# wangsibovictor/fora

Hardware: AMD Instinct MI355X
Metric: SSPPR queries/sec at eps=0.5 (higher is better)
Workload: dtype u64 fixed-point 2^-62 (f64 at the boundary)

## Files before the change

### fora_amd/csrc/fora_kernels.h

```cpp
#pragma once
#include <hip/hip_runtime.h>
#include <stdint.h>
#include <type_traits>
#include "fora_diag.h"

namespace fora {

constexpr int BLOCK = 256;
constexpr uint32_t PUSH_SEG = 256;
constexpr uint32_t WALK_SEG = 1024;
#ifndef FORA_TEST_PATHS
#define FORA_TEST_PATHS 0
#endif
constexpr bool TEST_PATHS = FORA_TEST_PATHS != 0;
constexpr uint64_t FIX_ONE = 1ull << 62;
constexpr uint32_t DEG_SAT = 0xFFFFFFu;
constexpr int MAX_LEVELS = 1 << 15;
#ifndef FORA_BIN_SHIFT
#define FORA_BIN_SHIFT 13
#endif
constexpr int BIN_SHIFT = FORA_BIN_SHIFT;
constexpr uint32_t BIN_SIZE = 1u << BIN_SHIFT;
#ifndef FORA_BIN_SHIFT_WIDE
#define FORA_BIN_SHIFT_WIDE 14
// ... 216 lines not shown
    if (r2 < 0) { q2--; r2 += b; }
    if (r2 >= (int64_t)b) { q2++; }
    return q1 + (uint64_t)q2;
}

__device__ __forceinline__ uint64_t node_thr(uint64_t t1, uint32_t deg) {
    if (deg == 0) return 1;
    uint64_t hi = __umul64hi(t1, (uint64_t)deg);
    return hi ? ~0ull : t1 * (uint64_t)deg;
}

__device__ __forceinline__ uint64_t pop_value(uint64_t afix, uint64_t r, uint32_t deg, uint64_t &res_add, uint64_t &dang) {
    const uint64_t keep = mulshift62(r, afix);
    const uint64_t push = r - keep;
    if (deg == 0) { res_add = keep; dang = push; return 0; }
    const uint64_t inc = div_u64_u32(push, deg);
    res_add = keep + (push - inc * deg);
    dang = 0;
    return inc;
}

__device__ __forceinline__ uint64_t thr_unit(uint64_t t1, uint32_t k) {
    return k == 0 ? t1 : ((t1 >> (63 - k)) ? (~0ull >> 1) : (t1 << k));
}

__device__ __forceinline__ void node_row(const Dev &d, uint32_t v, int64_t &beg, uint64_t &deg) {
    uint64_t ri = d.rowinfo[v];
    beg = (int64_t)(ri >> 24);
    deg = ri & DEG_SAT;
    if (deg == DEG_SAT) deg = (uint64_t)(d.row_ptr[v + 1] - beg);
}

__device__ __forceinline__ uint32_t ri_deg(const Dev &d, uint64_t ri, uint32_t v) {
    const uint32_t dg = (uint32_t)ri & DEG_SAT;
    return dg == DEG_SAT ? (uint32_t)(d.row_ptr[v + 1] - (int64_t)(ri >> 24)) : dg;
}

struct __attribute__((packed, aligned(4))) U32Pair { uint32_t a, b; };
__device__ __forceinline__ uint32_t colp_at(const Dev &d, uint64_t e) {
    uint32_t word, sh;
    if (d.colp32) {
        const uint32_t at = d.colbits * (uint32_t)e;
        word = at >> 5; sh = at & 31;
    } else {
        const uint64_t at = (uint64_t)d.colbits * e;
        word = (uint32_t)(at >> 5); sh = (uint32_t)at & 31;
    }
    const U32Pair cw = *(const U32Pair *)(d.colp + word);
    const uint64_t both = ((uint64_t)cw.b << 32) | cw.a;
    return (uint32_t)(both >> sh) & ((1u << d.colbits) - 1u);
}
__device__ __forceinline__ uint32_t walk_move(const Dev &d, uint32_t cur, uint32_t start, uint32_t wm) {
    if (d.rp32) {
        const U32Pair rp = *(const U32Pair *)(d.rp32 + cur);
        const uint32_t dg = rp.b - rp.a;
        if (!dg) return start;
        return colp_at(d, (uint64_t)rp.a + __umulhi(wm, dg));
    }
    int64_t beg; uint64_t deg;
    node_row(d, cur, beg, deg);
    if (!deg) return start;
    return (uint32_t)d.col[beg + (int64_t)(((uint64_t)wm * deg) >> 32)];
}

__device__ __forceinline__ uint64_t wave_sum(uint64_t v) {
#pragma unroll
    for (int o = 32; o; o >>= 1) v += __shfl_xor(v, o);
    return v;
}
template <int CTRL, int ROWS = 0xF>
__device__ __forceinline__ uint32_t dpp0(uint32_t x) { return (uint32_t)__builtin_amdgcn_update_dpp(0, (int)x, CTRL, ROWS, 0xF, false); }
__device__ __forceinline__ uint32_t wave_incl_scan_add(uint32_t x) {
    x += dpp0<0x111>(x); x += dpp0<0x112>(x); x += dpp0<0x114>(x); x += dpp0<0x118>(x);
    x += dpp0<0x142, 0xA>(x);
    x += dpp0<0x143, 0xC>(x);
    return x;
}
__device__ __forceinline__ uint32_t wave_incl_scan_max(uint32_t x) {
    x = max(x, dpp0<0x111>(x)); x = max(x, dpp0<0x112>(x)); x = max(x, dpp0<0x114>(x)); x = max(x, dpp0<0x118>(x));
    x = max(x, dpp0<0x142, 0xA>(x));
    x = max(x, dpp0<0x143, 0xC>(x));
    return x;
}
__device__ __forceinline__ uint32_t wave_excl_scan(uint32_t v, uint32_t &total) {
    const uint32_t x = wave_incl_scan_add(v);
    total = (uint32_t)__builtin_amdgcn_readlane((int)x, 63);
    return x - v;
}
template <int NT>
__device__ __forceinline__ uint32_t block_excl_scan_n(uint32_t v, uint32_t *s_w, uint32_t &total) {
    uint32_t wtot;
    uint32_t x = wave_excl_scan(v, wtot);
    const int w = threadIdx.x >> 6;
    __syncthreads();
    if ((threadIdx.x & 63) == 0) s_w[w] = wtot;
    __syncthreads();
    uint32_t before = 0, tot = 0;
#pragma unroll
    for (int i = 0; i < NT / 64; i++) { const uint32_t c = s_w[i]; if (i < w) before += c; tot += c; }
    total = tot;
    return x + before;
}
__device__ __forceinline__ uint32_t block_excl_scan(uint32_t v, uint32_t *s_w, uint32_t &total) {
    uint32_t wtot;
    uint32_t x = wave_excl_scan(v, wtot);
    const int w = threadIdx.x >> 6;
    __syncthreads();
    if ((threadIdx.x & 63) == 0) s_w[w] = wtot;
    __syncthreads();
    uint32_t a0 = s_w[0], a1 = s_w[1], a2 = s_w[2], a3 = s_w[3];
    total = a0 + a1 + a2 + a3;
    return x + (w > 0 ? a0 : 0) + (w > 1 ? a1 : 0) + (w > 2 ? a2 : 0);
}

constexpr int ilog2(int x) { return x <= 1 ? 0 : 1 + ilog2(x >> 1); }
template <int NT>
__device__ __forceinline__ uint32_t pref_find(const uint32_t *s_pref, uint32_t x) {
    static_assert((NT & (NT - 1)) == 0, "a power of two entries");
    uint32_t lo = 0, hi = NT;
#pragma unroll
    for (int it = 0; it < ilog2(NT); it++) {
        const uint32_t mid = (lo + hi) >> 1;
        if (s_pref[mid] <= x) lo = mid; else hi = mid;
    }
    return lo;
}
__device__ __forceinline__ uint32_t pref_step(const uint32_t *s_pref, uint32_t lo, uint32_t x) {
    while (s_pref[lo + 1] <= x) lo++;
    return lo;
}

template <typename T>
__device__ __forceinline__ void slab_load(uint64_t (&x)[SLAB_UNROLL], const uint64_t *p, T base, T v0, T step, T n) {
#pragma unroll
    for (int u = 0; u < SLAB_UNROLL; u++) x[u] = v0 + u * step < n ? p[base + v0 + u * step] : 0;
}

__device__ __forceinline__ void wave_append(bool flag, uint64_t item, uint64_t *list,
                                            unsigned long long *count, uint64_t cap, uint32_t *err,
                                            uint32_t errbit) {
    const unsigned long long mask = __ballot(flag);
    if (!mask) return;
    const int lane = threadIdx.x & 63;
    const int leader = __ffsll((long long)mask) - 1;
    unsigned long long base = 0;
    if (lane == leader) base = atomicAdd(count, (unsigned long long)__popcll(mask));
    base = __shfl(base, leader);
    if (flag) {
        uint64_t idx = base + __popcll(mask & ((1ull << lane) - 1));
        if (idx < cap) list[idx] = item;
        else atomicOr(err, errbit);
    }
}

__device__ __forceinline__ void wave_append32(bool flag, uint32_t item, uint32_t *list, uint32_t *count,
                                              uint32_t cap, uint32_t *err, uint32_t errbit) {
    const unsigned long long mask = __ballot(flag);
    if (!mask) return;
    const int lane = threadIdx.x & 63;
    const int leader = __ffsll((long long)mask) - 1;
    uint32_t base = 0;
    if (lane == leader) base = atomicAdd(count, (uint32_t)__popcll(mask));
    base = __shfl(base, leader);
    if (flag) {
        const uint32_t idx = base + __popcll(mask & ((1ull << lane) - 1));
        if (idx < cap) list[idx] = item;
// ... 1580 lines not shown
    }
    if (__ballot(bad) && (threadIdx.x & 63) == 0) atomicOr(&fail[q], 2u);
}
__global__ void __launch_bounds__(BLOCK) k_bounds_reset(int32_t n, double *upper, double *lower) {
    const uint64_t slab = (uint64_t)blockIdx.y * n;
    for (uint64_t v = (uint64_t)blockIdx.x * BLOCK + threadIdx.x; v < (uint64_t)n; v += (uint64_t)gridDim.x * BLOCK) {
        upper[slab + v] = 1.0;
        lower[slab + v] = 0.0;
    }
}

__global__ void __launch_bounds__(BLOCK) k_index_alloc(Dev d) {
    const int lane = threadIdx.x & 63;
    const int q = 0;
    const uint32_t nchunk = ((uint32_t)d.n + BLOCK - 1) / BLOCK;
    for (uint32_t c = blockIdx.x; c < nchunk; c += gridDim.x) {
        const uint32_t v = c * BLOCK + threadIdx.x;
        uint64_t num = 0, ioff = 0;
        if (v < (uint32_t)d.n) { num = d.idx_cnt[v]; ioff = d.idx_off[v]; }
        const uint32_t nseg = (uint32_t)((num + WALK_SEG - 1) / WALK_SEG);
        uint32_t tot;
        const uint32_t off = wave_excl_scan(nseg, tot);
        if (tot) {
            uint32_t sb = 0;
            if (lane == 0) sb = atomicAdd(&d.wit_count[q * CSTRIDE], tot);
            sb = __shfl(sb, 0);
            if ((uint64_t)sb + tot > d.wit_cap) {
                if (lane == 0) atomicOr(d.err, ERR_WIT_OVERFLOW);
            } else {
                for (uint32_t k = 0; k < nseg; k++) {
                    WalkItem w = {};
                    w.j0 = (uint64_t)k * WALK_SEG;
                    const uint64_t left = num - w.j0;
                    w.cnt = left < WALK_SEG ? (uint32_t)left : WALK_SEG;
                    w.idx_pos = ioff + w.j0;
                    w.v = v;
                    d.wit[sb + off + k] = wit_pack(w);
                }
            }
        }
    }
}

enum { WALK_TO_PPR = 0, WALK_TO_INDEX = 1 };

__device__ __forceinline__ int32_t walk_one(const Dev &d, uint32_t start, uint64_t j, uint32_t stream,
                                            uint32_t round, int nzh, uint32_t &steps) {
    int64_t beg; uint64_t deg;
    node_row(d, start, beg, deg);
    if (deg == 0) return (int32_t)start;
    uint32_t cur = start;
    uint32_t w[4];
    for (uint32_t t = 0;; t++) {
        if ((t & 1u) == 0)
            philox4x32_10(start, (uint32_t)j,
                          (uint32_t)((j >> 32) & 0xFFFFu) | ((round & 0xFFu) << 16) | (((t >> 1) & 0xFFu) << 24),
                          stream ^ ((t >> 9) * 0x9E3779B9u), d.seed_lo, d.seed_hi, w);
        const uint32_t ws = (t & 1u) ? w[2] : w[0], wm = (t & 1u) ? w[3] : w[1];
        if (!(nzh && t == 0) && ws < d.alpha32) return (int32_t)cur;
        if (t) node_row(d, cur, beg, deg);
        if (deg > 0)
            cur = (uint32_t)d.col[beg + (int64_t)(((uint64_t)wm * deg) >> 32)];
        else
            cur = start;
        steps++;
    }
}

#ifndef FORA_STAGE
#define FORA_STAGE 320
#endif
#ifndef FORA_WALK_WPE
#define FORA_WALK_WPE 6
#endif
constexpr int STAGE = FORA_STAGE;
struct WaveStage {
    uint64_t *pk;
    uint32_t *bcnt;
    uint32_t *bbase;
    uint32_t *fill;
    uint32_t count;
    const uint32_t *xl;
};
template <int ST>
__device__ __forceinline__ void stage_flush(const Dev &d, int q, WaveStage &st) {
    const int lane = threadIdx.x & 63;
    const uint64_t slab = (uint64_t)q * d.n;
    const uint64_t bk0 = SubBuckets::first_of(d.pbins, d.sub, d.bk_cap, q, blockIdx.x), bstride = SubBuckets::stride_of(d.sub, d.bk_cap);
    st.bcnt[lane] = 0;
    st.bcnt[lane + 64] = 0;
    __builtin_amdgcn_wave_barrier();
    constexpr uint64_t NONE = ~0ull;
    uint32_t rk[ST / 64];
    uint64_t wv[ST / 64];
#pragma unroll
    for (int k = 0; k < ST / 64; k++) {
        const uint32_t m = k * 64 + lane;
        wv[k] = NONE;
        if (m < st.count) {
            wv[k] = st.pk[m];
            rk[k] = atomicAdd(&st.bcnt[((uint32_t)wv[k] & ((1u << WPACK_SHIFT) - 1)) >> BIN_SHIFT], 1u);
        }
    }
    __builtin_amdgcn_wave_barrier();
    {
        const uint32_t c0 = lane < d.nbins ? st.bcnt[lane] : 0, c1 = lane + 64 < d.nbins ? st.bcnt[lane + 64] : 0;
        uint32_t t0, t1;
        const uint32_t o0 = wave_excl_scan(c0, t0), o1 = wave_excl_scan(c1, t1);
        if (c0) st.bbase[lane] = atomicAdd(&st.fill[lane], c0);
        if (c1) st.bbase[lane + 64] = atomicAdd(&st.fill[lane + 64], c1);
        st.bcnt[lane] = o0;
        st.bcnt[lane + 64] = t0 + o1;
    }
    __builtin_amdgcn_wave_barrier();
#pragma unroll
    for (int k = 0; k < ST / 64; k++)
        if (wv[k] != NONE) st.pk[st.bcnt[((uint32_t)wv[k] & ((1u << WPACK_SHIFT) - 1)) >> BIN_SHIFT] + rk[k]] = wv[k];
    __builtin_amdgcn_wave_barrier();
#pragma unroll
    for (int k = 0; k < ST / 64; k++) {
        const uint32_t m = k * 64 + lane;
        if (m < st.count) {
            const uint64_t pk = st.pk[m];
            const uint32_t dd = (uint32_t)pk & ((1u << WPACK_SHIFT) - 1);
            const uint32_t b = dd >> BIN_SHIFT;
            const uint32_t pos = st.bbase[b] + (m - st.bcnt[b]);
            if (pos < d.bk_cap) __builtin_nontemporal_store(pk, &d.bk_inc[bk0 + (uint64_t)b * bstride + pos]);
            else atomicAdd((unsigned long long *)&d.ppr[slab + (st.xl ? st.xl[dd] : dd)], (unsigned long long)(pk >> WPACK_SHIFT));
        }
    }
    __builtin_amdgcn_wave_barrier();
    st.count = 0;
}
template <int ST>
__device__ __forceinline__ void stage_emit(const Dev &d, int q, WaveStage &st, bool has, uint32_t dest, uint64_t w) {
    if (has && w >= WPACK_MAXW) {
        atomicAdd((unsigned long long *)&d.ppr[(uint64_t)q * d.n + (st.xl ? st.xl[dest] : dest)], (unsigned long long)w);
        has = false;
    }
    const unsigned long long mask = __ballot(has);
    if (!mask) return;
    if (has) {
        const uint32_t pos = st.count + __popcll(mask & ((1ull << (threadIdx.x & 63)) - 1));
        st.pk[pos] = (uint64_t)dest | (w << WPACK_SHIFT);
    }
    st.count += (uint32_t)__popcll(mask);
    if (st.count > ST - 64) stage_flush<ST>(d, q, st);
}
#define WAVE_STAGE_DECL_N(st, NWAVES, ST)                                                           \
    __shared__ uint64_t st##_pk[NWAVES][ST];                                                        \
    __shared__ uint32_t st##_bcnt[NWAVES][MAX_BINS], st##_bbase[NWAVES][MAX_BINS];                 \
    __shared__ uint32_t st##_fill[MAX_BINS];                                                        \
    WaveStage st;                                                                                   \
    st.pk = st##_pk[threadIdx.x >> 6];                                                              \
    st.bcnt = st##_bcnt[threadIdx.x >> 6]; st.bbase = st##_bbase[threadIdx.x >> 6];                 \
    st.fill = st##_fill; st.count = 0; st.xl = nullptr;
#define WAVE_STAGE_DECL(st) WAVE_STAGE_DECL_N(st, BLOCK / 64, STAGE)

template <int NB>
__global__ void __launch_bounds__(BinThreads<NB>::value) k_walk_idx(Dev d) {
    constexpr int NT = BinThreads<NB>::value;
    constexpr int EPT = NB > MAX_BINS ? FORA_IDX_EPT_WIDE : BIN_EPT;
    constexpr uint32_t CHUNK = NT * EPT;
    constexpr uint32_t PAD = NB > MAX_BINS ? FORA_RUN_PAD_WIDE : 1;
    constexpr bool BINNED = NB > 1;
    constexpr bool WIDE = NB > MAX_BINS;
    constexpr int BS = WIDE ? BIN_SHIFT_WIDE : BIN_SHIFT;
    constexpr uint32_t BSZ = 1u << BS;
    constexpr int IB = NT == 256 ? 8 : NT == 512 ? 9 : 10;
    constexpr int DB = WIDE ? BS : WPACK_SHIFT;
    static_assert(DB + IB + 1 <= 32, "stage word: destination | item | carries-one-more-unit");
    __shared__ uint64_t s_j0[NT], s_pos[NT], s_incr[NT], s_rem[NT];
    __shared__ uint32_t s_pref[NT + 1], s_w[NT / 64];
    __shared__ uint32_t s_cnt[NB], s_lofs[NB + 1], s_fill[NB];
    __shared__ uint32_t s_msg[BINNED ? CHUNK : 1];
    __shared__ uint16_t s_bin[BINNED ? CHUNK : 1];
    const bool slot_major = NB > MAX_BINS && (d.slot_major & 4u);
    const int q = slot_major ? blockIdx.x : blockIdx.y;
    const uint32_t bx = slot_major ? blockIdx.y : blockIdx.x, gx = slot_major ? gridDim.y : gridDim.x;
    const uint32_t nitems = (uint32_t)min((uint64_t)d.wit_count[q * CSTRIDE], d.wit_cap);
    if (!nitems || *d.err) return;
    const WalkItemP *items = d.wit + (uint64_t)q * d.wit_cap;
    const uint64_t slab = (uint64_t)q * d.n;
    const uint32_t bin_lo = (uint32_t)d.bin_lo;
    const BinExchange<NB, NT, PAD> ex{s_cnt, s_lofs, s_fill, s_w, SubBuckets(d.bk_count, d.pbins, d.sub, d.bk_cap, q, bx), (uint32_t)d.bin_cnt};
    if (BINNED) ex.load_fills();
    constexpr uint32_t GRAN = FORA_TILE_GRAN_WALK;
    const uint32_t ntiles = (nitems + NT - 1) / NT;
    const uint32_t seg_len = ntiles * GRAN;
    for (uint32_t tile = bx; tile < ntiles; tile += gx) {
        const uint32_t i = tile_pos<GRAN>(threadIdx.x, tile, seg_len);
        uint32_t cnt = 0;
        if (i < nitems) {
            const WalkItem w = wit_load(&items[i]);
            s_j0[threadIdx.x] = w.j0; s_pos[threadIdx.x] = w.idx_pos;
            s_incr[threadIdx.x] = w.incr; s_rem[threadIdx.x] = w.rem;
            cnt = w.idx_n;
        }
        uint32_t total;
        const uint32_t pre = block_excl_scan_n<NT>(cnt, s_w, total);
        s_pref[threadIdx.x] = pre;
        if (threadIdx.x == 0) s_pref[NT] = total;
        __syncthreads();
        for (uint32_t cb = 0; cb < total; cb += CHUNK) {
            uint32_t dest[EPT], rank[EPT], li[EPT];
            const uint32_t e0 = cb + threadIdx.x * EPT;
            uint32_t lo = e0 < total ? pref_find<NT>(s_pref, e0) : 0;
#pragma unroll
            for (int k = 0; k < EPT; k++) {
                const uint32_t e = e0 + k;
                if (e < total) lo = pref_step(s_pref, lo, e);
                li[k] = lo;
            }
#pragma unroll
            for (int k = 0; k < EPT; k++) {
                const uint32_t e = e0 + k;
                dest[k] = 0xFFFFFFFFu;
                if (e < total) {
                    const uint32_t jj = e - s_pref[li[k]];
                    dest[k] = (uint32_t)d.rw_idx[s_pos[li[k]] + jj];
                    li[k] |= (s_j0[li[k]] + jj < s_rem[li[k]] ? 1u : 0u) << IB;
                }
            }
            if (!BINNED) {
#pragma unroll
                for (int k = 0; k < EPT; k++)
                    if (dest[k] != 0xFFFFFFFFu)
                        atomicAdd((unsigned long long *)&d.ppr[slab + dest[k]],
                                  (unsigned long long)(s_incr[li[k] & (NT - 1)] + (li[k] >> IB)));
                continue;
// ... 114 lines not shown
                    }
                    const uint32_t want = (uint32_t)__popcll(idle);
                    wptr += want < avail ? want : avail;
                    while (wptr < wend && s_pref[cur_item + 1] <= wptr) cur_item++;
                }
                if (active)
                    philox4x32_10(start, (uint32_t)wj,
                                  (uint32_t)((wj >> 32) & 0xFFFFu) | ((round & 0xFFu) << 16) | (((t >> 1) & 0xFFu) << 24),
                                  stream ^ ((t >> 9) * 0x9E3779B9u), d.seed_lo, d.seed_hi, rw);
            }
            if (active) {
                const uint32_t ws = (it & 1u) ? rw[2] : rw[0], wm = (it & 1u) ? rw[3] : rw[1];
                if (!(nzh && t == 0) && ws < d.alpha32) {
                    done = (int32_t)cur;
                    active = false;
                } else {
                    if (t) cur = walk_move(d, cur, start, wm);
                    else if (d.rp32) cur = colp_at(d, (uint64_t)beg0 + (((uint64_t)wm * deg0) >> 32));
                    else cur = (uint32_t)d.col[beg0 + (int64_t)(((uint64_t)wm * deg0) >> 32)];
                    t++;
                    steps++;
                }
            }
            if (staged) {
                stage_emit<STAGE>(d, q, st, done >= 0, (uint32_t)done, wgt);
            } else if (done >= 0) {
                if (MODE == WALK_TO_INDEX) idx_out[opos] = done;
                else atomicAdd((unsigned long long *)&d.ppr[slab + (uint32_t)done], (unsigned long long)wgt);
            }
        }
        __syncthreads();
    }
    if (staged && st.count) stage_flush<STAGE>(d, q, st);
    if (staged) {
        __syncthreads();
        for (uint32_t i = threadIdx.x; i < (uint32_t)d.nbins; i += BLOCK) bkc[(uint64_t)i * d.sub] = st.fill[i];
    }
    const uint64_t ws = wave_sum((uint64_t)steps);
    __syncthreads();
    if ((threadIdx.x & 63) == 0) s_w[threadIdx.x >> 6] = (uint32_t)ws;
    __syncthreads();
    if (threadIdx.x == 0) {
        const unsigned long long bs = (unsigned long long)s_w[0] + s_w[1] + s_w[2] + s_w[3];
        if (bs) atomicAdd(d.tot_steps, bs);
    }
}

#ifndef FORA_DG_THREADS
#define FORA_DG_THREADS 512
#endif
#ifndef FORA_DG_STAGE
#define FORA_DG_STAGE 256
#endif
#ifndef FORA_DG_WPE
#define FORA_DG_WPE 6
#endif
constexpr int DG_THREADS = FORA_DG_THREADS;
constexpr int DG_STAGE = FORA_DG_STAGE;
#ifndef FORA_DG_TILE
#define FORA_DG_TILE 256
#endif
constexpr int DG_TILE = FORA_DG_TILE;
typedef uint32_t __attribute__((aligned(1))) u32_unaligned;
template <bool BITS32>
__device__ __forceinline__ uint32_t dg_colp_at(const WalkDG &g, uint32_t e) {
    if (BITS32) {
        const uint32_t at = g.bits * e;
        const uint32_t w = *(const u32_unaligned *)((const char *)g.colp + (at >> 3));
        return (w >> (at & 7)) & ((1u << g.bits) - 1u);
    }
    uint32_t word, sh;
    if (BITS32) { const uint32_t at = g.bits * e; word = at >> 5; sh = at & 31; }
    else { const uint64_t at = (uint64_t)g.bits * e; word = (uint32_t)(at >> 5); sh = (uint32_t)at & 31; }
    const U32Pair cw = *(const U32Pair *)(g.colp + word);
    const uint64_t both = ((uint64_t)cw.b << 32) | cw.a;
    return (uint32_t)(both >> sh) & ((1u << g.bits) - 1u);
}
template <bool NZH, bool BITS32, bool XL>
__global__ void __launch_bounds__(DG_THREADS) __attribute__((amdgpu_waves_per_eu(FORA_DG_WPE, 8))) k_walk_dg(Dev d, uint32_t round) {
    constexpr int NW = DG_THREADS / 64;
    extern __shared__ __attribute__((aligned(16))) uint64_t dg_lds64[];
    constexpr int WT = DG_TILE / NW;
    static_assert(WT >= 1 && WT <= 64, "a lane loads one item of its wave's tile");
    __shared__ uint64_t w_j0[NW][WT], w_incr[NW][WT], w_rem[NW][WT];
    __shared__ uint32_t w_v[NW][WT], w_vp[NW][WT], w_idxn[NW][WT], w_pref[NW][WT + 1], s_w[NW];
    __shared__ unsigned long long w_self[XL ? NW : 1][XL ? WT : 1];
    const int q = blockIdx.y;
    const uint32_t nitems = (uint32_t)min((uint64_t)d.wit_count[q * CSTRIDE], d.wit_cap);
    if (!nitems || *d.err) return;
    const WalkDG &g = d.dg;
    const uint32_t H = g.H, ts = g.ts, nblk1 = g.nblk ? g.nblk - 1 : 0;
    unsigned long long *s_hub = (unsigned long long *)dg_lds64;
    uint32_t *dg_lds = (uint32_t *)(dg_lds64 + (XL ? ((H + 1) & ~1u) : 0));
    uint4 *s_rec = (uint4 *)dg_lds;
    const uint8_t *s_T = (const uint8_t *)(dg_lds + 4 * g.nrec);
    for (uint32_t i = threadIdx.x; i < g.nrec; i += DG_THREADS) s_rec[i] = make_uint4(g.rec[i], g.rec[g.nrec + i], g.rec[2 * g.nrec + i], 0u);
    for (uint32_t i = threadIdx.x; i < (g.nblk + 3) / 4; i += DG_THREADS) dg_lds[4 * g.nrec + i] = ((const uint32_t *)g.T)[i];
    if (XL) for (uint32_t i = threadIdx.x; i < H; i += DG_THREADS) s_hub[i] = 0;
    const WalkItemP *items = d.wit + (uint64_t)q * d.wit_cap;
    const uint64_t slab = (uint64_t)q * d.n;
    const uint32_t stream = (uint32_t)d.src[q];
    const int lane = threadIdx.x & 63, wid = threadIdx.x >> 6;
    uint32_t steps = 0;
    WAVE_STAGE_DECL_N(st, NW, DG_STAGE)
    if (XL) st.xl = g.invb;
    uint32_t *bkc = d.bk_count + (uint64_t)q * d.pbins * d.sub + blockIdx.x;
    for (uint32_t i = threadIdx.x; i < (uint32_t)MAX_BINS; i += DG_THREADS) st.fill[i] = i < (uint32_t)d.nbins ? bkc[(uint64_t)i * d.sub] : 0;
    __syncthreads();
    auto move = [&](uint32_t cur, uint32_t startp, uint32_t wm) -> uint32_t {
        const uint32_t tb = s_T[min((cur - H) >> ts, nblk1)];
        const uint32_t r = cur < H ? cur : H + tb;
        const uint4 rc = s_rec[r];
        const uint32_t dg = rc.y;
        const uint32_t e = rc.z + (cur - rc.x) * dg + __umulhi(wm, dg);
        const uint32_t nx = dg_colp_at<BITS32>(g, dg ? e : 0u);
        return dg ? nx : startp;
    };
    bool pend = false;
    uint32_t pend_node = 0;
    uint64_t pend_w = 0;
    unsigned long long *s_self = w_self[XL ? wid : 0];
    if (XL && lane < WT) s_self[lane] = 0;
    uint32_t gen = 0, tag = 0;
    auto flush_self = [&]() {
        if (!XL) return;
        const unsigned long long sv = lane < WT ? s_self[lane] : 0ull;
        const uint32_t dn = lane < WT ? w_vp[wid][lane] : 0u;
        if (lane < WT && sv) s_self[lane] = 0;
        if (sv && dn < H) atomicAdd(&s_hub[dn], sv);
        const uint32_t u = dn - H, blk = u >> 6;
        const uint32_t qd = __umulhi(blk, g.nbx_magic);
        const uint32_t dest = ((blk - qd * g.nbx) << BIN_SHIFT) | (qd << 6) | (u & 63u);
        stage_emit<DG_STAGE>(d, q, st, sv != 0 && dn >= H, dest, (uint64_t)sv);
    };
    uint64_t *s_j0 = w_j0[wid], *s_incr = w_incr[wid], *s_rem = w_rem[wid];
    uint32_t *s_v = w_v[wid], *s_vp = w_vp[wid], *s_idxn = w_idxn[wid], *s_pref = w_pref[wid];
    const uint32_t ntiles = (nitems + WT - 1) / WT;
    uint32_t tile = blockIdx.x * NW + wid;
    const uint32_t tstride = gridDim.x * NW;
    uint32_t wptr = 0, wend = 0;
    uint32_t cur_item = 0;
    bool active = false;
    uint32_t cur = 0, start = 0, startp = 0, t = 0;
    uint64_t wj = 0, wgt = 0;
    for (;;) {
        int32_t done = -1;
        const unsigned long long idle = __ballot(!active);
        if (idle && wptr == wend) {
            while (wptr == wend && tile < ntiles) {
                if (gen) flush_self();
                gen++;
                const uint32_t i = tile * WT + lane;
                uint32_t cnt = 0;
                if (lane < WT && i < nitems) {
                    WalkItem w;
                    {
                        const uint64_t *wp = (const uint64_t *)&items[i];
                        const uint64_t x0 = NT_LOAD(wp), x1 = NT_LOAD(wp + 1), x3 = NT_LOAD(wp + 3);
                        w = wit_unpack(x0, x1, 0, x3);
                    }
                    s_j0[lane] = w.j0; s_incr[lane] = w.incr; s_rem[lane] = w.rem;
                    s_v[lane] = w.v;
                    s_vp[lane] = g.perm[w.v];
                    s_idxn[lane] = w.idx_n;
                    cnt = w.cnt - w.idx_n;
                }
                uint32_t total;
                const uint32_t pre = wave_excl_scan(cnt, total);
                if (lane < WT) s_pref[lane] = pre;
                if (lane == 0) s_pref[WT] = total;
                __builtin_amdgcn_fence(__ATOMIC_RELEASE, "wavefront");
                __builtin_amdgcn_wave_barrier();
                wptr = 0; wend = total; cur_item = 0;
                tile += tstride;
                while (wptr < wend && (uint32_t)__builtin_amdgcn_readfirstlane((int)s_pref[cur_item + 1]) <= wptr) cur_item++;
            }
        }
        const uint32_t avail = wend - wptr;
        if (!avail && idle == ~0ull) break;
        if (avail && idle) {
            const uint32_t rank = __popcll(idle & ((1ull << lane) - 1));
            if (!active && rank < avail) {
                const uint32_t e = wptr + rank;
                uint32_t item = cur_item;
                while (s_pref[item + 1] <= e) item++;
                const uint32_t jj = s_idxn[item] + (e - s_pref[item]);
                wj = s_j0[item] + jj;
                start = s_v[item];
                startp = s_vp[item];
                wgt = s_incr[item] + (wj < s_rem[item] ? 1 : 0);
                cur = startp;
                t = 0;
                tag = (gen << 6) | item;
                if (startp >= g.zero_first) done = (int32_t)startp;
                else active = true;
            }
            const uint32_t want = (uint32_t)__popcll(idle);
            wptr += want < avail ? want : avail;
            while (wptr < wend && (uint32_t)__builtin_amdgcn_readfirstlane((int)s_pref[cur_item + 1]) <= wptr) cur_item++;
            __builtin_amdgcn_wave_barrier();
        }
        if (active) {
            uint32_t rw[4];
            philox4x32_10(start, (uint32_t)wj,
                          (uint32_t)((wj >> 32) & 0xFFFFu) | ((round & 0xFFu) << 16) | (((t >> 1) & 0xFFu) << 24),
                          stream ^ ((t >> 9) * 0x9E3779B9u), d.seed_lo, d.seed_hi, rw);
            if (!(NZH && t == 0) && rw[0] < d.alpha32) {
                done = (int32_t)cur;
                active = false;
            } else {
                cur = move(diag::dg_from(cur, t), startp, rw[1]);
                steps++;
                if (rw[2] < d.alpha32) {
                    t++;
                    done = (int32_t)cur;
                    active = false;
                } else {
                    cur = move(diag::dg_from(cur, 1u), startp, rw[3]);
                    t += 2;
                    steps++;
                }
            }
        }
        if (XL) {
            bool ended = done >= 0;
            const uint32_t dn = (uint32_t)done;
            if (ended && dn == startp && (tag >> 6) == gen) {
                atomicAdd(&s_self[tag & 63u], (unsigned long long)wgt);
                ended = false;
            }
            if (ended && dn < H) atomicAdd(&s_hub[dn], (unsigned long long)wgt);
            const uint32_t u = dn - H, blk = u >> 6;
            const uint32_t qd = __umulhi(blk, g.nbx_magic);
            const uint32_t dest = ((blk - qd * g.nbx) << BIN_SHIFT) | (qd << 6) | (u & 63u);
            stage_emit<DG_STAGE>(d, q, st, ended && dn >= H, dest, wgt);
        } else {
            stage_emit<DG_STAGE>(d, q, st, pend, pend_node, pend_w);
            pend = done >= 0;
            if (pend) { pend_node = g.inv[done]; pend_w = wgt; }
        }
    }
    if (!XL) stage_emit<DG_STAGE>(d, q, st, pend, pend_node, pend_w);
    if (gen) flush_self();
    if (st.count) stage_flush<DG_STAGE>(d, q, st);
    __syncthreads();
    for (uint32_t i = threadIdx.x; i < (uint32_t)d.nbins; i += DG_THREADS) bkc[(uint64_t)i * d.sub] = st.fill[i];
    if (XL) for (uint32_t i = threadIdx.x; i < H; i += DG_THREADS) {
        const unsigned long long hv = s_hub[i];
        if (hv) atomicAdd((unsigned long long *)&d.ppr[slab + g.inv[i]], hv);
    }
    const uint64_t ws = wave_sum((uint64_t)steps);
    if (lane == 0) s_w[wid] = (uint32_t)ws;
    __syncthreads();
    if (threadIdx.x == 0) {
        unsigned long long bs = 0;
#pragma unroll
        for (int w = 0; w < NW; w++) bs += s_w[w];
        if (bs) atomicAdd(d.tot_steps, bs);
    }
}

__global__ void __launch_bounds__(BLOCK) k_ppr_sum(Dev d) {
    const int q = blockIdx.y;
    const uint64_t slab = (uint64_t)q * d.n;
    uint64_t acc = 0;
    const uint64_t step = (uint64_t)gridDim.x * BLOCK;
    for (uint64_t v0 = (uint64_t)blockIdx.x * BLOCK + threadIdx.x; v0 < (uint64_t)d.n; v0 += step * SLAB_UNROLL) {
        uint64_t x[SLAB_UNROLL];
        slab_load(x, d.ppr, slab, v0, step, (uint64_t)d.n);
#pragma unroll
        for (int u = 0; u < SLAB_UNROLL; u++) acc += x[u];
    }
    acc = wave_sum(acc);
    if ((threadIdx.x & 63) == 0 && acc) atomicAdd(&d.qs[q].ppr_sum, (unsigned long long)acc);
}

__global__ void __launch_bounds__(BLOCK) k_walk_counts_f64(int32_t n, const double *residue, double rsum,
                                                           double omega, double alpha, int opt,
                                                           uint64_t *num_s_rw, uint64_t *n_rw) {
    double check_rsum = rsum;
    if (opt) check_rsum *= (1 - alpha);
    const uint64_t N = check_rsum == 0.0 ? 0 : (uint64_t)(omega * check_rsum);
    const int v = blockIdx.x * BLOCK + threadIdx.x;
    if (v == 0) *n_rw = N;
    if (v >= n) return;
    double r = residue[v];
    uint64_t num = 0;
    if (r > 0 && check_rsum != 0.0) {
        if (opt) r = r * (1 - alpha);
        num = walk_count(r, check_rsum, N);
    }
    num_s_rw[v] = num;
}

__global__ void __launch_bounds__(BLOCK) k_walks_raw(Dev d, uint32_t stream, uint32_t round, int nzh,
                                                     const int32_t *starts, const uint64_t *js, int64_t count,
                                                     int32_t *dests) {
    const int64_t i = (int64_t)blockIdx.x * BLOCK + threadIdx.x;
    if (i >= count) return;
    uint32_t steps = 0;
    dests[i] = walk_one(d, (uint32_t)starts[i], js[i], stream, round, nzh, steps);
}

constexpr int MC_TAB_BITS = 11;
constexpr uint32_t MC_TAB = 1u << MC_TAB_BITS;
constexpr int MC_PROBES = 8;
constexpr uint32_t MC_EMPTY = 0xFFFFFFFFu;
__device__ __forceinline__ bool mc_tab_add(uint32_t *keys, unsigned long long *vals, uint32_t v, uint64_t w) {
    uint32_t h = (v * 0x9E3779B1u) >> (32 - MC_TAB_BITS);
    for (int p = 0; p < MC_PROBES; p++) {
        uint32_t k = keys[h];
        if (k == MC_EMPTY) {
            k = atomicCAS(&keys[h], MC_EMPTY, v);
            if (k == MC_EMPTY) k = v;
        }
        if (k == v) {
            atomicAdd(&vals[h], (unsigned long long)w);
            return true;
        }
        h = (h + 1) & (MC_TAB - 1);
    }
    return false;
}
__global__ void __launch_bounds__(BLOCK) k_walk_mc(Dev d, uint64_t wbase, uint64_t wrem, uint64_t j0, uint64_t j1, uint64_t per_wg) {
    __shared__ uint32_t s_key[MC_TAB];
    __shared__ unsigned long long s_val[MC_TAB];
    __shared__ unsigned long long s_src[BLOCK / 64];
// ... 10 lines not shown
        beg0 = rp.a;
        deg0 = rp.b - rp.a;
    } else node_row(d, s, beg0, deg0);
    if (deg0 == 0) {
        if (threadIdx.x == 0) {
            const uint64_t extra = wrem > lo ? min(hi, wrem) - lo : 0;
            atomicAdd((unsigned long long *)&d.ppr[slab + s], (unsigned long long)((hi - lo) * wbase + extra));
        }
        return;
    }
    for (uint32_t i = threadIdx.x; i < MC_TAB; i += BLOCK) { s_key[i] = MC_EMPTY; s_val[i] = 0; }
    __syncthreads();
    const int lane = threadIdx.x & 63, wid = threadIdx.x >> 6;
    const uint64_t span = hi - lo;
    uint64_t wptr = lo + ((span * (uint64_t)wid) >> 2);
    const uint64_t wend = lo + ((span * (uint64_t)(wid + 1)) >> 2);
    bool active = false;
    uint32_t cur = s, t = 0, steps = 0;
    uint64_t wj = 0, src_acc = 0;
    uint32_t rw[4] = {0, 0, 0, 0};
    for (uint32_t it = 0;; it++) {
        if ((it & 1u) == 0) {
            const unsigned long long idle = __ballot(!active);
            const uint64_t avail = wend - wptr;
            if (!avail && idle == ~0ull) break;
            if (avail && idle) {
                const uint32_t rank = __popcll(idle & ((1ull << lane) - 1));
                if (!active && rank < avail) {
                    wj = wptr + rank;
                    cur = s;
                    t = 0;
                    active = true;
                }
                const uint32_t want = (uint32_t)__popcll(idle);
                wptr += want < avail ? want : avail;
            }
            if (active)
                philox4x32_10(s, (uint32_t)wj, (uint32_t)((wj >> 32) & 0xFFFFu) | (((t >> 1) & 0xFFu) << 24),
                              s ^ ((t >> 9) * 0x9E3779B9u), d.seed_lo, d.seed_hi, rw);
        }
        if (active) {
            const uint32_t ws = (it & 1u) ? rw[2] : rw[0], wm = (it & 1u) ? rw[3] : rw[1];
            if (ws < d.alpha32) {
                active = false;
                const uint64_t w = wbase + (wj < wrem ? 1u : 0u);
                if (cur == s) src_acc += w;
                else if (!mc_tab_add(s_key, s_val, cur, w)) atomicAdd((unsigned long long *)&d.ppr[slab + cur], (unsigned long long)w);
            } else {
                if (t) cur = walk_move(d, cur, s, wm);
                else if (d.rp32) cur = colp_at(d, (uint64_t)beg0 + (((uint64_t)wm * deg0) >> 32));
                else cur = (uint32_t)d.col[beg0 + (int64_t)(((uint64_t)wm * deg0) >> 32)];
                t++;
                steps++;
            }
        }
    }
    const uint64_t ssum = wave_sum(src_acc), wsteps = wave_sum((uint64_t)steps);
    if (lane == 0) { s_src[wid] = ssum; s_steps[wid] = (uint32_t)wsteps; }
    __syncthreads();
    for (uint32_t i = threadIdx.x; i < MC_TAB; i += BLOCK) {
        const uint32_t v = s_key[i];
        if (v != MC_EMPTY) atomicAdd((unsigned long long *)&d.ppr[slab + v], s_val[i]);
    }
    if (threadIdx.x == 0) {
        unsigned long long a = 0, b = 0;
        for (int w = 0; w < BLOCK / 64; w++) { a += s_src[w]; b += s_steps[w]; }
        if (a) atomicAdd((unsigned long long *)&d.ppr[slab + s], a);
        if (b) atomicAdd(d.tot_steps, b);
    }
}

constexpr int SP_TILE = 2 * BLOCK;
constexpr int SP_UNROLL = 4;
__device__ __forceinline__ void sp_load(const uint64_t *slab, int64_t p, int64_t lo, int64_t hi, uint64_t &a, uint64_t &b) {
    a = 0; b = 0;
    if (p >= lo && p + 1 < hi) {
        const ulonglong2 x = *reinterpret_cast<const ulonglong2 *>(slab + p);
        a = x.x; b = x.y;
    } else {
        if (p >= lo && p < hi) a = slab[p];
        if (p + 1 >= lo && p + 1 < hi) b = slab[p + 1];
    }
}
__device__ __forceinline__ uint32_t sp_mbcnt(unsigned long long mask) {
    return __builtin_amdgcn_mbcnt_hi((uint32_t)(mask >> 32), __builtin_amdgcn_mbcnt_lo((uint32_t)mask, 0u));
}
__global__ void __launch_bounds__(BLOCK) k_sparse_count(const uint64_t *ppr, uint32_t n, uint64_t thr, uint32_t R, uint32_t *counts,
                                                        uint32_t *tot) {
    __shared__ uint32_t s_w[BLOCK / 64];
    const uint32_t q = blockIdx.y;
    const uint64_t first = (uint64_t)q * n;
    const uint64_t *slab = ppr + first;
    const int64_t lo = (int64_t)blockIdx.x * R, hi = min((int64_t)n, lo + (int64_t)R);
    uint32_t c = 0;
    const auto masked = [&](int64_t t) {
        uint64_t a, b;
        sp_load(slab, t + 2 * (int64_t)threadIdx.x, lo, hi, a, b);
        c += (a >= thr ? 1u : 0u) + (b >= thr ? 1u : 0u);
    };
    int64_t t = lo - (int64_t)(first & 1);
    if (first & 1) { masked(t); t += SP_TILE; }
    for (; t + (int64_t)SP_TILE * SP_UNROLL <= hi; t += (int64_t)SP_TILE * SP_UNROLL) {
        const ulonglong2 *src = reinterpret_cast<const ulonglong2 *>(slab + t) + threadIdx.x;
        ulonglong2 x[SP_UNROLL];
#pragma unroll
        for (int u = 0; u < SP_UNROLL; u++) x[u] = src[u * BLOCK];
#pragma unroll
        for (int u = 0; u < SP_UNROLL; u++) c += (x[u].x >= thr ? 1u : 0u) + (x[u].y >= thr ? 1u : 0u);
    }
    for (; t < hi; t += SP_TILE) masked(t);
    c = (uint32_t)wave_sum((uint64_t)c);
    if ((threadIdx.x & 63) == 0) s_w[threadIdx.x >> 6] = c;
    __syncthreads();
    if (threadIdx.x == 0) {
        uint32_t t = 0;
#pragma unroll
        for (int w = 0; w < BLOCK / 64; w++) t += s_w[w];
        counts[(uint64_t)q * gridDim.x + blockIdx.x] = t;
        if (t) atomicAdd(&tot[q], t);
    }
}
__global__ void __launch_bounds__(BLOCK) k_sparse_write(const uint64_t *ppr, uint32_t n, uint64_t thr, uint32_t R, const uint32_t *counts,
                                                        const int64_t *base, int32_t *ids, uint64_t *fix, uint64_t cap) {
    __shared__ uint32_t s_w[2][BLOCK / 64];
    __shared__ uint32_t s_before[BLOCK / 64];
    const uint32_t q = blockIdx.y;
    const uint32_t *cq = counts + (uint64_t)q * gridDim.x;
    const uint32_t mine = cq[blockIdx.x];
    if (!mine) return;
    const int lane = threadIdx.x & 63, w = threadIdx.x >> 6;
    uint32_t part = 0;
    for (uint32_t x = threadIdx.x; x < blockIdx.x; x += BLOCK) part += cq[x];
    part = (uint32_t)wave_sum((uint64_t)part);
    if (lane == 0) s_before[w] = part;
    __syncthreads();
    uint32_t before = 0;
#pragma unroll
    for (int i = 0; i < BLOCK / 64; i++) before += s_before[i];
    uint64_t out = (uint64_t)base[q] + before;
    const uint64_t first = (uint64_t)q * n;
    const uint64_t *slab = ppr + first;
    const int64_t lo = (int64_t)blockIdx.x * R, hi = min((int64_t)n, lo + (int64_t)R);
    int64_t p = lo - (int64_t)(first & 1) + 2 * (int64_t)threadIdx.x;
    uint64_t a, b;
    sp_load(slab, p, lo, hi, a, b);
    uint32_t done = 0;
    for (int64_t t = lo - (int64_t)(first & 1); t < hi && done < mine; t += SP_TILE, p += SP_TILE) {
        const int par = (int)((uint64_t)(t - lo + 1) / SP_TILE) & 1;
        uint64_t na, nb;
        sp_load(slab, p + SP_TILE, lo, hi, na, nb);
        const bool fa = a >= thr, fb = b >= thr;
        const unsigned long long ma = __ballot(fa), mb = __ballot(fb);
        const uint32_t rank = sp_mbcnt(ma) + sp_mbcnt(mb);
        if (lane == 0) s_w[par][w] = (uint32_t)(__popcll(ma) + __popcll(mb));
        __syncthreads();
        uint32_t off = rank, tile = 0;
#pragma unroll
        for (int i = 0; i < BLOCK / 64; i++) { const uint32_t c = s_w[par][i]; if (i < w) off += c; tile += c; }
        const uint64_t ia = out + off, ib = ia + (fa ? 1u : 0u);
        if (fa && ia < cap) { ids[ia] = (int32_t)p; fix[ia] = a; }
        if (fb && ib < cap) { ids[ib] = (int32_t)(p + 1); fix[ib] = b; }
        out += tile; done += tile;
        a = na; b = nb;
    }
}
__global__ void __launch_bounds__(BLOCK) k_sparse_single(uint32_t cnt, const int64_t *at, const int32_t *src, int32_t *ids, uint64_t *fix, uint64_t cap) {
    const uint32_t i = blockIdx.x * BLOCK + threadIdx.x;
    if (i < cnt && (uint64_t)at[i] < cap) { ids[at[i]] = src[i]; fix[at[i]] = FIX_ONE; }
}
// ... 79 lines not shown
```

Baseline: 6772.

## Streamline degree-grouped walk kernel inner loop and defer destination remapping to flush

Reworks the k_walk_dg inner loop. Tile items are packed into one 32-byte LDS struct read with two vector loads, and the per-step philox counter is kept as incrementally updated words instead of being recomputed from t. Hub records are reordered so the move lookup needs no clamp or select, and the bin-destination remap is moved from every emit into stage_flush under a template flag. Overweight-check branches are skipped unless the tile contains big weights, and popcount rank is replaced with mbcnt. The aim is to cut VALU work and register pressure per walk step, at the cost of subtle counter-encoding and ordering logic that must stay bit-exact.

```diff
diff --git a/fora_amd/csrc/fora_kernels.h b/fora_amd/csrc/fora_kernels.h
--- a/fora_amd/csrc/fora_kernels.h
+++ b/fora_amd/csrc/fora_kernels.h
@@ -322,6 +322,9 @@
     x = max(x, dpp0<0x143, 0xC>(x));
     return x;
 }
+__device__ __forceinline__ uint32_t sp_mbcnt(unsigned long long mask) {
+    return __builtin_amdgcn_mbcnt_hi((uint32_t)(mask >> 32), __builtin_amdgcn_mbcnt_lo((uint32_t)mask, 0u));
+}
 __device__ __forceinline__ uint32_t wave_excl_scan(uint32_t v, uint32_t &total) {
     const uint32_t x = wave_incl_scan_add(v);
     total = (uint32_t)__builtin_amdgcn_readlane((int)x, 63);
@@ -2068,7 +2071,7 @@
     uint32_t count;
     const uint32_t *xl;
 };
-template <int ST>
+template <int ST, bool XLD = false>
 __device__ __forceinline__ void stage_flush(const Dev &d, int q, WaveStage &st) {
     const int lane = threadIdx.x & 63;
     const uint64_t slab = (uint64_t)q * d.n;
@@ -2085,6 +2088,12 @@
         wv[k] = NONE;
         if (m < st.count) {
             wv[k] = st.pk[m];
+            if (XLD) {
+                const uint32_t lo = (uint32_t)wv[k], u = lo & ((1u << WPACK_SHIFT) - 1), blk = u >> 6;
+                const uint32_t qd = __umulhi(blk, d.dg.nbx_magic);
+                const uint32_t dest = ((blk - qd * d.dg.nbx) << BIN_SHIFT) | (qd << 6) | (u & 63u);
+                wv[k] = (wv[k] & 0xFFFFFFFF00000000ull) | ((lo & ~((1u << WPACK_SHIFT) - 1)) | dest);
+            }
             rk[k] = atomicAdd(&st.bcnt[((uint32_t)wv[k] & ((1u << WPACK_SHIFT) - 1)) >> BIN_SHIFT], 1u);
         }
     }
@@ -2118,20 +2127,20 @@
     __builtin_amdgcn_wave_barrier();
     st.count = 0;
 }
-template <int ST>
+template <int ST, bool XLD = false, bool CHECKW = true>
 __device__ __forceinline__ void stage_emit(const Dev &d, int q, WaveStage &st, bool has, uint32_t dest, uint64_t w) {
-    if (has && w >= WPACK_MAXW) {
+    if (CHECKW && has && w >= WPACK_MAXW) {
         atomicAdd((unsigned long long *)&d.ppr[(uint64_t)q * d.n + (st.xl ? st.xl[dest] : dest)], (unsigned long long)w);
         has = false;
     }
     const unsigned long long mask = __ballot(has);
     if (!mask) return;
     if (has) {
-        const uint32_t pos = st.count + __popcll(mask & ((1ull << (threadIdx.x & 63)) - 1));
+        const uint32_t pos = st.count + sp_mbcnt(mask);
         st.pk[pos] = (uint64_t)dest | (w << WPACK_SHIFT);
     }
     st.count += (uint32_t)__popcll(mask);
-    if (st.count > ST - 64) stage_flush<ST>(d, q, st);
+    if (st.count > ST - 64) stage_flush<ST, XLD>(d, q, st);
 }
 #define WAVE_STAGE_DECL_N(st, NWAVES, ST)                                                           \
     __shared__ uint64_t st##_pk[NWAVES][ST];                                                        \
@@ -2412,25 +2421,28 @@
     extern __shared__ __attribute__((aligned(16))) uint64_t dg_lds64[];
     constexpr int WT = DG_TILE / NW;
     static_assert(WT >= 1 && WT <= 64, "a lane loads one item of its wave's tile");
-    __shared__ uint64_t w_j0[NW][WT], w_incr[NW][WT], w_rem[NW][WT];
-    __shared__ uint32_t w_v[NW][WT], w_vp[NW][WT], w_idxn[NW][WT], w_pref[NW][WT + 1], s_w[NW];
+    struct __attribute__((aligned(16))) TileItem { uint64_t jb, rem, incr; uint32_t v, vp; };
+    static_assert(sizeof(TileItem) == 32, "two uint4");
+    __shared__ TileItem w_item[NW][WT];
+    __shared__ uint32_t w_pref[NW][WT + 1], s_w[NW];
     __shared__ unsigned long long w_self[XL ? NW : 1][XL ? WT : 1];
     const int q = blockIdx.y;
     const uint32_t nitems = (uint32_t)min((uint64_t)d.wit_count[q * CSTRIDE], d.wit_cap);
     if (!nitems || *d.err) return;
     const WalkDG &g = d.dg;
-    const uint32_t H = g.H, ts = g.ts, nblk1 = g.nblk ? g.nblk - 1 : 0;
+    const uint32_t H = g.H, ts = g.ts;
     unsigned long long *s_hub = (unsigned long long *)dg_lds64;
     uint32_t *dg_lds = (uint32_t *)(dg_lds64 + (XL ? ((H + 1) & ~1u) : 0));
     uint4 *s_rec = (uint4 *)dg_lds;
+    const uint32_t ncls = g.nrec - H;
     const uint8_t *s_T = (const uint8_t *)(dg_lds + 4 * g.nrec);
-    for (uint32_t i = threadIdx.x; i < g.nrec; i += DG_THREADS) s_rec[i] = make_uint4(g.rec[i], g.rec[g.nrec + i], g.rec[2 * g.nrec + i], 0u);
+    for (uint32_t i = threadIdx.x; i < g.nrec; i += DG_THREADS) s_rec[i < H ? ncls + i : i - H] = make_uint4(g.rec[i], g.rec[g.nrec + i], g.rec[2 * g.nrec + i], 0u);
     for (uint32_t i = threadIdx.x; i < (g.nblk + 3) / 4; i += DG_THREADS) dg_lds[4 * g.nrec + i] = ((const uint32_t *)g.T)[i];
     if (XL) for (uint32_t i = threadIdx.x; i < H; i += DG_THREADS) s_hub[i] = 0;
     const WalkItemP *items = d.wit + (uint64_t)q * d.wit_cap;
     const uint64_t slab = (uint64_t)q * d.n;
     const uint32_t stream = (uint32_t)d.src[q];
-    const int lane = threadIdx.x & 63, wid = threadIdx.x >> 6;
+    const int lane = threadIdx.x & 63, wid = __builtin_amdgcn_readfirstlane((int)(threadIdx.x >> 6));
     uint32_t steps = 0;
     WAVE_STAGE_DECL_N(st, NW, DG_STAGE)
     if (XL) st.xl = g.invb;
@@ -2438,141 +2450,150 @@
     for (uint32_t i = threadIdx.x; i < (uint32_t)MAX_BINS; i += DG_THREADS) st.fill[i] = i < (uint32_t)d.nbins ? bkc[(uint64_t)i * d.sub] : 0;
     __syncthreads();
     auto move = [&](uint32_t cur, uint32_t startp, uint32_t wm) -> uint32_t {
-        const uint32_t tb = s_T[min((cur - H) >> ts, nblk1)];
-        const uint32_t r = cur < H ? cur : H + tb;
+        uint32_t r = ncls + cur;
+        if (cur >= H) r = s_T[(cur - H) >> ts];
         const uint4 rc = s_rec[r];
         const uint32_t dg = rc.y;
         const uint32_t e = rc.z + (cur - rc.x) * dg + __umulhi(wm, dg);
-        const uint32_t nx = dg_colp_at<BITS32>(g, dg ? e : 0u);
+        const uint32_t nx = dg_colp_at<BITS32>(g, e);
         return dg ? nx : startp;
     };
     bool pend = false;
     uint32_t pend_node = 0;
     uint64_t pend_w = 0;
     unsigned long long *s_self = w_self[XL ? wid : 0];
+    TileItem *s_item = w_item[wid];
+    uint32_t *s_pref = w_pref[wid];
     if (XL && lane < WT) s_self[lane] = 0;
     uint32_t gen = 0, tag = 0;
     auto flush_self = [&]() {
         if (!XL) return;
         const unsigned long long sv = lane < WT ? s_self[lane] : 0ull;
-        const uint32_t dn = lane < WT ? w_vp[wid][lane] : 0u;
+        const uint32_t dn = lane < WT ? s_item[lane].vp : 0u;
         if (lane < WT && sv) s_self[lane] = 0;
         if (sv && dn < H) atomicAdd(&s_hub[dn], sv);
-        const uint32_t u = dn - H, blk = u >> 6;
-        const uint32_t qd = __umulhi(blk, g.nbx_magic);
-        const uint32_t dest = ((blk - qd * g.nbx) << BIN_SHIFT) | (qd << 6) | (u & 63u);
-        stage_emit<DG_STAGE>(d, q, st, sv != 0 && dn >= H, dest, (uint64_t)sv);
+        bool has = sv != 0 && dn >= H;
+        if (has && sv >= WPACK_MAXW) {
+            atomicAdd((unsigned long long *)&d.ppr[slab + g.inv[dn]], sv);
+            has = false;
+        }
+        stage_emit<DG_STAGE, true, false>(d, q, st, has, dn - H, (uint64_t)sv);
     };
-    uint64_t *s_j0 = w_j0[wid], *s_incr = w_incr[wid], *s_rem = w_rem[wid];
-    uint32_t *s_v = w_v[wid], *s_vp = w_vp[wid], *s_idxn = w_idxn[wid], *s_pref = w_pref[wid];
     const uint32_t ntiles = (nitems + WT - 1) / WT;
     uint32_t tile = blockIdx.x * NW + wid;
     const uint32_t tstride = gridDim.x * NW;
     uint32_t wptr = 0, wend = 0;
     uint32_t cur_item = 0;
+    bool big = false;
+    auto advance = [&]() {
+        while (wptr < wend && (uint32_t)__builtin_amdgcn_readfirstlane((int)s_pref[cur_item + 1]) <= wptr) cur_item++;
+    };
     bool active = false;
-    uint32_t cur = 0, start = 0, startp = 0, t = 0;
-    uint64_t wj = 0, wgt = 0;
+    uint32_t cur = 0, start = 0, startp = 0, c1 = 0, c2 = 0, c3 = 0;
+    const uint32_t c2_round = (round & 0xFFu) << 16;
+    uint64_t wgt = 0;
     for (;;) {
-        int32_t done = -1;
+        bool fin = false;
         const unsigned long long idle = __ballot(!active);
         if (idle && wptr == wend) {
             while (wptr == wend && tile < ntiles) {
                 if (gen) flush_self();
                 gen++;
                 const uint32_t i = tile * WT + lane;
-                uint32_t cnt = 0;
-                if (lane < WT && i < nitems) {
-                    WalkItem w;
-                    {
-                        const uint64_t *wp = (const uint64_t *)&items[i];
-                        const uint64_t x0 = NT_LOAD(wp), x1 = NT_LOAD(wp + 1), x3 = NT_LOAD(wp + 3);
-                        w = wit_unpack(x0, x1, 0, x3);
-                    }
-                    s_j0[lane] = w.j0; s_incr[lane] = w.incr; s_rem[lane] = w.rem;
-                    s_v[lane] = w.v;
-                    s_vp[lane] = g.perm[w.v];
-                    s_idxn[lane] = w.idx_n;
-                    cnt = w.cnt - w.idx_n;
-                }
+                const bool have = lane < WT && i < nitems;
+                WalkItem w = {};
+                if (have) {
+                    const uint64_t *wp = (const uint64_t *)&items[i];
+                    const uint64_t x0 = NT_LOAD(wp), x1 = NT_LOAD(wp + 1), x3 = NT_LOAD(wp + 3);
+                    w = wit_unpack(x0, x1, 0, x3);
+                }
+                const uint32_t cnt = have ? w.cnt - w.idx_n : 0u;
                 uint32_t total;
                 const uint32_t pre = wave_excl_scan(cnt, total);
+                if (have) {
+                    TileItem it;
+                    it.jb = w.j0 + w.idx_n - pre;
+                    it.rem = w.rem; it.incr = w.incr;
+                    it.v = w.v; it.vp = g.perm[w.v];
+                    s_item[lane] = it;
+                }
+                if (__ballot(have && w.incr + 1 >= WPACK_MAXW)) big = true;
                 if (lane < WT) s_pref[lane] = pre;
                 if (lane == 0) s_pref[WT] = total;
                 __builtin_amdgcn_fence(__ATOMIC_RELEASE, "wavefront");
                 __builtin_amdgcn_wave_barrier();
                 wptr = 0; wend = total; cur_item = 0;
                 tile += tstride;
-                while (wptr < wend && (uint32_t)__builtin_amdgcn_readfirstlane((int)s_pref[cur_item + 1]) <= wptr) cur_item++;
+                advance();
             }
         }
         const uint32_t avail = wend - wptr;
         if (!avail && idle == ~0ull) break;
         if (avail && idle) {
-            const uint32_t rank = __popcll(idle & ((1ull << lane) - 1));
+            const uint32_t rank = sp_mbcnt(idle);
             if (!active && rank < avail) {
                 const uint32_t e = wptr + rank;
                 uint32_t item = cur_item;
                 while (s_pref[item + 1] <= e) item++;
-                const uint32_t jj = s_idxn[item] + (e - s_pref[item]);
-                wj = s_j0[item] + jj;
-                start = s_v[item];
-                startp = s_vp[item];
-                wgt = s_incr[item] + (wj < s_rem[item] ? 1 : 0);
+                const uint4 ia = ((const uint4 *)&s_item[item])[0], ib = ((const uint4 *)&s_item[item])[1];
+                const uint64_t wj = (((uint64_t)ia.y << 32) | ia.x) + e;
+                const uint64_t rem = ((uint64_t)ia.w << 32) | ia.z;
+                wgt = (((uint64_t)ib.y << 32) | ib.x) + (wj < rem ? 1 : 0);
+                start = ib.z;
+                startp = ib.w;
+                c1 = (uint32_t)wj;
+                c2 = ((uint32_t)(wj >> 32) & 0xFFFFu) | c2_round;
+                c3 = stream;
                 cur = startp;
-                t = 0;
                 tag = (gen << 6) | item;
-                if (startp >= g.zero_first) done = (int32_t)startp;
-                else active = true;
+                fin = startp >= g.zero_first;
+                active = !fin;
             }
             const uint32_t want = (uint32_t)__popcll(idle);
             wptr += want < avail ? want : avail;
-            while (wptr < wend && (uint32_t)__builtin_amdgcn_readfirstlane((int)s_pref[cur_item + 1]) <= wptr) cur_item++;
+            advance();
             __builtin_amdgcn_wave_barrier();
         }
         if (active) {
             uint32_t rw[4];
-            philox4x32_10(start, (uint32_t)wj,
-                          (uint32_t)((wj >> 32) & 0xFFFFu) | ((round & 0xFFu) << 16) | (((t >> 1) & 0xFFu) << 24),
-                          stream ^ ((t >> 9) * 0x9E3779B9u), d.seed_lo, d.seed_hi, rw);
-            if (!(NZH && t == 0) && rw[0] < d.alpha32) {
-                done = (int32_t)cur;
-                active = false;
+            philox4x32_10(start, c1, c2, c3, d.seed_lo, d.seed_hi, rw);
+            const uint32_t later = (c2 >> 24) | (c3 ^ stream);
+            c2 += 1u << 24;
+            if (__ballot(c2 < (1u << 24))) {
+                asm volatile("" ::: "memory");
+                if (c2 < (1u << 24)) c3 = stream ^ ((c3 ^ stream) + 0x9E3779B9u);
+            }
+            if (!(NZH && later == 0) && rw[0] < d.alpha32) {
+                fin = true;
             } else {
-                cur = move(diag::dg_from(cur, t), startp, rw[1]);
+                cur = move(diag::dg_from(cur, later), startp, rw[1]);
                 steps++;
                 if (rw[2] < d.alpha32) {
-                    t++;
-                    done = (int32_t)cur;
-                    active = false;
+                    fin = true;
                 } else {
                     cur = move(diag::dg_from(cur, 1u), startp, rw[3]);
-                    t += 2;
                     steps++;
                 }
             }
+            active = !fin;
         }
         if (XL) {
-            bool ended = done >= 0;
-            const uint32_t dn = (uint32_t)done;
-            if (ended && dn == startp && (tag >> 6) == gen) {
-                atomicAdd(&s_self[tag & 63u], (unsigned long long)wgt);
-                ended = false;
-            }
-            if (ended && dn < H) atomicAdd(&s_hub[dn], (unsigned long long)wgt);
-            const uint32_t u = dn - H, blk = u >> 6;
-            const uint32_t qd = __umulhi(blk, g.nbx_magic);
-            const uint32_t dest = ((blk - qd * g.nbx) << BIN_SHIFT) | (qd << 6) | (u & 63u);
-            stage_emit<DG_STAGE>(d, q, st, ended && dn >= H, dest, wgt);
+            const bool self = fin && cur == startp && tag >= (gen << 6);
+            if (self) atomicAdd(&s_self[tag & 63u], (unsigned long long)wgt);
+            const bool away = fin && !self;
+            if (away && cur < H) atomicAdd(&s_hub[cur], (unsigned long long)wgt);
+            const bool over = big && wgt >= WPACK_MAXW;
+            if (away && cur >= H && over) atomicAdd((unsigned long long *)&d.ppr[slab + g.inv[cur]], (unsigned long long)wgt);
+            stage_emit<DG_STAGE, true, false>(d, q, st, away && cur >= H && !over, cur - H, wgt);
         } else {
             stage_emit<DG_STAGE>(d, q, st, pend, pend_node, pend_w);
-            pend = done >= 0;
-            if (pend) { pend_node = g.inv[done]; pend_w = wgt; }
+            pend = fin;
+            if (pend) { pend_node = g.inv[cur]; pend_w = wgt; }
         }
     }
     if (!XL) stage_emit<DG_STAGE>(d, q, st, pend, pend_node, pend_w);
     if (gen) flush_self();
-    if (st.count) stage_flush<DG_STAGE>(d, q, st);
+    if (st.count) stage_flush<DG_STAGE, XL>(d, q, st);
     __syncthreads();
     for (uint32_t i = threadIdx.x; i < (uint32_t)d.nbins; i += DG_THREADS) bkc[(uint64_t)i * d.sub] = st.fill[i];
     if (XL) for (uint32_t i = threadIdx.x; i < H; i += DG_THREADS) {
@@ -2749,9 +2770,6 @@
         if (p + 1 >= lo && p + 1 < hi) b = slab[p + 1];
     }
 }
-__device__ __forceinline__ uint32_t sp_mbcnt(unsigned long long mask) {
-    return __builtin_amdgcn_mbcnt_hi((uint32_t)(mask >> 32), __builtin_amdgcn_mbcnt_lo((uint32_t)mask, 0u));
-}
 __global__ void __launch_bounds__(BLOCK) k_sparse_count(const uint64_t *ppr, uint32_t n, uint64_t thr, uint32_t R, uint32_t *counts,
                                                         uint32_t *tot) {
     __shared__ uint32_t s_w[BLOCK / 64];
```

New measurement: 6902, median of 6. +1.9%, better.
